# yzh119/custom_op_benchmark

Measured on AMD Instinct MI355X. Metric: edges/sec fwd+bwd (SDDMM+softmax+SpMM) on Reddit d=64; HBM GB/s vs roofline, higher is better.
Workload: dtype f32; 1 GPU; reddit-shape Chung-Lu(alpha=0.50) graph, N=232965 E=114615892 per GPU, h=1 d=64, U[0,1) values, chunk_size=32, int64 CSR both orientations; graph=reddit, nodes=232965, edges=114615892, heads=1, d=64, chunk_size=32, row_chunks=3694777, col_chunks=3694424, parallelism=single GPU

## Files before the change

### custom_op_benchmark_amd/_lib.py

```python
import atexit
import collections
import ctypes
import os
import weakref

import torch

_HERE = os.path.dirname(os.path.abspath(__file__))
LIB_PATH = os.environ.get("GRAPHOP_LIB") or os.path.join(_HERE, "libgraphop_hip.so")
ABI_VERSION = 8

F32, F64 = 0, 1
_c64 = ctypes.c_int64
_vp = ctypes.c_void_p
_lib = None


class PlanInfo(ctypes.Structure):
    _fields_ = [("n_chunks", _c64), ("n_edges", _c64), ("n_segments", _c64), ("max_row", _c64),
                ("max_index", _c64), ("max_segment_len", _c64), ("rows_sorted", ctypes.c_int32),
                ("indptr_monotone", ctypes.c_int32), ("eid_identity", ctypes.c_int32),
                ("full_coverage", ctypes.c_int32), ("row_owned", ctypes.c_int32),
                ("has_idx32", ctypes.c_int32), ("dense_fill_pct", ctypes.c_int32),
                ("sorted_in_rows", ctypes.c_int32), ("n_dense_blocks", _c64), ("max_row_gap", _c64),
                ("n_geometry_fallbacks", _c64),
                ("sddmm_tile_rows", ctypes.c_int32), ("sddmm_tile_repeat_permille", ctypes.c_int32),
                ("sddmm_tile_max_parts", ctypes.c_int32)]


class SweepInfo(ctypes.Structure):
    _fields_ = [("win_cols", _c64), ("W", ctypes.c_int32), ("T", ctypes.c_int32), ("V", ctypes.c_int32),
                ("n_dealt", ctypes.c_int32)]


ALLOC_FN = ctypes.CFUNCTYPE(ctypes.c_void_p, ctypes.c_size_t, ctypes.c_int, ctypes.c_void_p)
FREE_FN = ctypes.CFUNCTYPE(None, ctypes.c_void_p)


class ProfileRec(ctypes.Structure):
    _fields_ = [("name", ctypes.c_char * 48), ("kernel", ctypes.c_char * 48), ("calls", _c64), ("total_ms", ctypes.c_double),
                ("min_ms", ctypes.c_double), ("max_ms", ctypes.c_double)]


_P = _vp
_SIGNATURES = {
    "graphop_tune": [ctypes.c_char_p, ctypes.c_int],
    "graphop_tune_reset": [],
    "graphop_check_device_errors": [],
    "graphop_tune_get": [ctypes.c_char_p, ctypes.POINTER(ctypes.c_int)],
    "graphop_profile_enable": [ctypes.c_int],
    "graphop_profile_read": [ctypes.POINTER(ProfileRec), ctypes.c_int],
    "graphop_partition_csr_count": [_P, _c64, _c64, _P, _P],
    "graphop_partition_csr_fill": [_P, _P, _c64, _c64, _c64, _P, _P, _P],
    "graphop_plan_create": [_P, _P, _P, _P, _c64, _c64, _c64, _P, ctypes.POINTER(_vp)],
    "graphop_plan_info": [_P, ctypes.POINTER(PlanInfo)],
    "graphop_set_allocator": [ALLOC_FN, FREE_FN],
    "graphop_plan_prepare": [_P, ctypes.c_int, _c64, _c64, _c64, ctypes.c_int, _P],
    "graphop_plan_n_sweeps": [_P],
    "graphop_plan_sweep_info": [_P, ctypes.c_int, ctypes.POINTER(SweepInfo)],
    "graphop_plan_array": [_P, ctypes.c_char_p, ctypes.c_int, ctypes.POINTER(_vp), ctypes.POINTER(_c64)],
    "graphop_plan_import": [_P] * 4 + [ctypes.POINTER(PlanInfo)] + [_P] * 4 + [_c64] + [_P] * 4 + [ctypes.POINTER(_vp)],
    "graphop_plan_import_sweep": [_P, ctypes.POINTER(SweepInfo), _P, _P, _P, _P],
    "graphop_plan_sweep_dealt": [_P, ctypes.c_int, ctypes.c_int, ctypes.POINTER(ctypes.c_int32), ctypes.POINTER(ctypes.c_int32)],
    "graphop_plan_sweep_build_dealt": [_P, ctypes.POINTER(SweepInfo), ctypes.c_int32, ctypes.c_int32, _P],
    "graphop_maskedmm_csr_forward": [ctypes.c_int] + [_P] * 7 + [_c64] * 6 + [_P, _P],
    "graphop_maskedmm_csr_forward_partial": [ctypes.c_int] + [_P] * 7 + [_c64] * 7 + [_P],
    "graphop_maskedmm_csr_backward": [ctypes.c_int] + [_P] * 13 + [_c64] * 7 + [_P, _P, _P],
    "graphop_sparse_softmax_forward": [ctypes.c_int] + [_P] * 5 + [_c64] * 3 + [_P, _c64, _P, _P],
    "graphop_sparse_softmax_backward": [ctypes.c_int] + [_P] * 6 + [_c64] * 3 + [_P, _c64, _P, _P],
    "graphop_vector_spmm_forward": [ctypes.c_int] + [_P] * 7 + [_c64] * 6 + [_P, _P],
    "graphop_vector_spmm_backward": [ctypes.c_int] + [_P] * 13 + [_c64] * 7 + [_P, _P, _P],
    "graphop_spmm_pair_supported": [ctypes.c_int] + [_c64] * 5 + [_P],
    "graphop_spmm_pair": [ctypes.c_int] + [_P] * 9 + [_c64] * 6 + [_P, _P],
    "graphop_interleave_pairs": [ctypes.c_int, _P, _P, _P, _c64, _P],
    "graphop_node_mul_edge_forward": [ctypes.c_int] + [_P] * 6 + [_c64] * 5 + [_P, _P],
    "graphop_node_mul_edge_backward": [ctypes.c_int] + [_P] * 8 + [_c64] * 5 + [_P, _P],
    "graphop_gat_scores_forward": [ctypes.c_int] + [_P] * 7 + [_c64] * 5 + [ctypes.c_double, _P, _P],
    "graphop_gat_scores_backward": [ctypes.c_int] + [_P] * 13 + [_c64] * 6 + [ctypes.c_double, _P, _P, _P],
    "graphop_gatv2_scores_forward": [ctypes.c_int] + [_P] * 8 + [_c64] * 6 + [ctypes.c_double, _P, _P],
    "graphop_gatv2_scores_backward": [ctypes.c_int] + [_P] * 16 + [_c64] * 8 + [ctypes.c_double, _P, _P, _P],
    "graphop_gatv2_attention_forward": [ctypes.c_int] + [_P] * 9 + [_c64] * 6 + [ctypes.c_double, _P, _P],
    "graphop_gatv2_attention_backward": [ctypes.c_int] + [_P] * 18 + [_c64] * 8 + [ctypes.c_double, _P, _P, _P],
    "graphop_gatv2_attention_dropout_forward": [ctypes.c_int] + [_P] * 9 + [_c64] * 6
    + [ctypes.c_double, ctypes.c_double, ctypes.c_uint64, ctypes.c_uint32, _P, _P],
    "graphop_gatv2_attention_dropout_backward": [ctypes.c_int] + [_P] * 18 + [_c64] * 8
    + [ctypes.c_double, ctypes.c_double, ctypes.c_uint64, ctypes.c_uint32, _P, _P, _P],
    "graphop_gat_attention_forward": [ctypes.c_int] + [_P] * 9 + [_c64] * 6 + [ctypes.c_double, _P, _P],
    "graphop_gat_attention_backward": [ctypes.c_int] + [_P] * 18 + [_c64] * 8 + [ctypes.c_double, _P, _P, _P],
    "graphop_gat_attention_dropout_forward": [ctypes.c_int] + [_P] * 9 + [_c64] * 6
    + [ctypes.c_double, ctypes.c_double, ctypes.c_uint64, ctypes.c_uint32, _P, _P],
    "graphop_gat_attention_dropout_backward": [ctypes.c_int] + [_P] * 18 + [_c64] * 8
    + [ctypes.c_double, ctypes.c_double, ctypes.c_uint64, ctypes.c_uint32, _P, _P, _P],
    "graphop_edge_dropout_mask": [ctypes.c_int] + [_P] * 5 + [_c64] * 5
    + [ctypes.c_double, ctypes.c_uint64, ctypes.c_uint32, _P, _P],
    "graphop_gat_edge_attention_forward": [ctypes.c_int] + [_P] * 10 + [_c64] * 6
    + [ctypes.c_double, ctypes.c_double, ctypes.c_uint64, ctypes.c_uint32, _P, _P],
    "graphop_gat_edge_attention_backward": [ctypes.c_int] + [_P] * 20 + [_c64] * 8
    + [ctypes.c_double, ctypes.c_double, ctypes.c_uint64, ctypes.c_uint32, _P, _P, _P],
    "graphop_gatv2_edge_attention_forward": [ctypes.c_int] + [_P] * 10 + [_c64] * 6
    + [ctypes.c_double, ctypes.c_double, ctypes.c_uint64, ctypes.c_uint32, _P, _P],
    "graphop_gatv2_edge_attention_backward": [ctypes.c_int] + [_P] * 20 + [_c64] * 8
    + [ctypes.c_double, ctypes.c_double, ctypes.c_uint64, ctypes.c_uint32, _P, _P, _P],
    "graphop_gather_rows": [ctypes.c_int, _P, _P, _P, _c64, _c64, _c64, _P],
    "graphop_scatter_add_rows": [ctypes.c_int, _P, _P, _P, _c64, _c64, _c64, _P],
    "graphop_add_rows_unique": [ctypes.c_int, _P, _P, _P, _c64, _c64, _c64, _P],
    "graphop_add_rows_grouped": [ctypes.c_int, _P, _P, _P, _P, _P, _c64, _c64, _c64, _P],
    "graphop_attention_workspace_bytes": [ctypes.c_int, ctypes.c_int] + [_c64] * 5 + [_P, _P, _P,
                                                                                       ctypes.POINTER(_c64)],
    "graphop_attention_backward_is_fused": [ctypes.c_int] + [_c64] * 5 + [_P, _P, _P, ctypes.POINTER(ctypes.c_int)],
    "graphop_attention_forward": [ctypes.c_int] + [_P] * 9 + [_c64] * 6 + [_P, _c64, _P, _P],
    "graphop_attention_backward": [ctypes.c_int] + [_P] * 17 + [_c64] * 7 + [_P, _c64, _P, _P, _P],
    "graphop_attention_dropout_workspace_bytes": [ctypes.c_int, ctypes.c_int] + [_c64] * 5 + [_P, _P, _P,
                                                                                               ctypes.POINTER(_c64)],
    "graphop_attention_dropout_forward": [ctypes.c_int] + [_P] * 9 + [_c64] * 6 + [_P, _c64, _P, _P]
    + [ctypes.c_double, ctypes.c_uint64, ctypes.c_uint32, _c64],
    "graphop_attention_dropout_backward": [ctypes.c_int] + [_P] * 17 + [_c64] * 7 + [_P, _c64, _P, _P, _P]
    + [ctypes.c_double, ctypes.c_uint64, ctypes.c_uint32, _c64],
    "graphop_attention_bias_workspace_bytes": [ctypes.c_int, ctypes.c_int] + [_c64] * 5 + [_P, _P, _P, ctypes.c_int,
                                                                                            ctypes.POINTER(_c64)],
    "graphop_attention_bias_forward": [ctypes.c_int] + [_P] * 10 + [_c64] * 6 + [_P, _c64, _P, _P]
    + [ctypes.c_double, ctypes.c_uint64, ctypes.c_uint32, _c64],
    "graphop_attention_bias_backward": [ctypes.c_int] + [_P] * 19 + [_c64] * 7 + [_P, _c64, _P, _P, _P]
    + [ctypes.c_double, ctypes.c_uint64, ctypes.c_uint32, _c64],
    "graphop_attention_edge_workspace_bytes": [ctypes.c_int, ctypes.c_int] + [_c64] * 5 + [_P, _P, _P,
                                                                                            ctypes.POINTER(_c64)],
    "graphop_attention_edge_forward": [ctypes.c_int] + [_P] * 10 + [_c64] * 6 + [_P, _c64, _P, _P]
    + [ctypes.c_double, ctypes.c_uint64, ctypes.c_uint32, _c64],
    "graphop_attention_edge_backward": [ctypes.c_int] + [_P] * 19 + [_c64] * 7 + [_P, _c64, _P, _P, _P]
    + [ctypes.c_double, ctypes.c_uint64, ctypes.c_uint32, _c64],
    "graphop_attention_etype_workspace_bytes": [ctypes.c_int, ctypes.c_int] + [_c64] * 6 + [_P, _P, _P,
                                                                                             ctypes.POINTER(_c64)],
    "graphop_attention_etype_forward": [ctypes.c_int] + [_P] * 11 + [_c64] * 7 + [_P, _c64, _P, _P]
    + [ctypes.c_double, ctypes.c_uint64, ctypes.c_uint32, _c64],
    "graphop_attention_etype_backward": [ctypes.c_int] + [_P] * 20 + [_c64] * 8 + [_P, _c64, _P, _P, _P]
    + [ctypes.c_double, ctypes.c_uint64, ctypes.c_uint32, _c64],
    "graphop_attention_tbias_workspace_bytes": [ctypes.c_int, ctypes.c_int] + [_c64] * 6 + [_P, _P, _P,
                                                                                             ctypes.POINTER(_c64)],
    "graphop_attention_tbias_forward": [ctypes.c_int] + [_P] * 11 + [_c64] * 7 + [_P, _c64, _P, _P]
    + [ctypes.c_double, ctypes.c_uint64, ctypes.c_uint32, _c64],
    "graphop_attention_tbias_backward": [ctypes.c_int] + [_P] * 20 + [_c64] * 8 + [_P, _c64, _P, _P, _P]
    + [ctypes.c_double, ctypes.c_uint64, ctypes.c_uint32, _c64],
# ... 418 lines not shown
```

### custom_op_benchmark_amd/csrc/graphop_hip.hip

```cpp
#include <stdarg.h>

#include <map>
#include <mutex>
#include <set>
#include <string>
#include <vector>

#include "common.h"
#include "host.h"
#include "host_attn_rows.h"
#include "kernels_fast.h"
#include "kernels_walk.h"
#include "kernels_tile.h"
#include "tile_layout.h"
#include "kernels_attn_walk.h"
#include "kernels_attn_bias_fwd.h"
#include "kernels_block.h"
#include "kernels_attn.h"
#include "kernels_generic.h"

namespace graphop {

namespace {

// ... 361 lines not shown
    } else {
      allow_full_lds((const void*)k_attn_fwd_walk_f32<L, false>);
      hipLaunchKernelGGL((k_attn_fwd_walk_f32<L, false>), dim3(wl.blocks), dim3(kWalkThreads), lds_bytes, st, wl.view, a, NoDrop{});
    }
  }
  attn_pieces_merge(
      "attn_fwd_merge", "k_attn_piece_add", w, L, st,
      [&](dim3 grid, dim3 block) { hipLaunchKernelGGL(k_attn_piece_max, grid, block, 0, st, w.p_row, w.p_ml, w.Mtmp, w.np); },
      [&](dim3 grid, dim3 block) {
        hipLaunchKernelGGL((k_attn_piece_add<L>), grid, block, 0, st, w.p_row, w.p_ml, w.p_o, w.Mtmp, w.Ltmp, a.o, w.np);
      },
      [&](dim3 grid, dim3 block) {
        hipLaunchKernelGGL((k_attn_piece_fin<L>), grid, block, 0, st, w.p_row, w.Mtmp, w.Ltmp, a.o, a.stats, w.np);
      });
  if (hipGetLastError() != hipSuccess) return -GRAPHOP_ERR_HIP;
  return 1;
}

int attn_bias_fwd_rows(const Csr& g, i64 n_q, i64 n_k, i64 h, i64 d, int dtype, const void* Q, const void* K,
                       const void* V, const void* b, void* o, void* stats, void* ws, i64 ws_bytes, hipStream_t st,
                       bool dry_run, size_t* ws_needed, const AttnDrop* drop) {
  const Tuning& t = tuning();
  const graphop_plan* plan = g.plan;
  const i64 n_chunks = g.n_chunks, n_edges = g.n_edges;
  if (ws_needed) *ws_needed = 0;
  if (!t.attn_fused || !t.attn_rows || t.force_generic || dtype != GRAPHOP_F32 || h != 1 || !plan) return 0;
  if (d % 4 != 0 || !pow2(d) || d < 16 || d > 1024 || n_edges == 0 || n_chunks == 0) return 0;
  if (!g.owned() || !plan->indices) return 0;
  if (plan->info.max_row >= n_q || plan->info.max_index >= n_k || n_q >= kWalkRowMask) return 0;
  const i64 F = d;
  const ChunkGeometry geo = attn_one_head_geometry(n_chunks, F);
  if (2 * geo.groups >= 0x7fffffffLL) return 0;
  const AttnRowsFwdWs w(ws, 2 * geo.groups, n_q, 1, F);
  if (ws_needed) *ws_needed = w.total;
  if (dry_run) return 1;
  if (!ws || (size_t)ws_bytes < w.total) return 0;
  AttnBiasFwdArgs a;
  a.Q = (const float*)Q; a.K = (const float*)K; a.V = (const float*)V; a.b = (const float*)b;
  a.o = (float*)o; a.stats = (float*)stats;
  a.p_row = w.p_row; a.p_ml = w.p_ml; a.p_o = w.p_o;
  if (zero_async(o, sizeof(float) * (size_t)(n_q * F), st) != hipSuccess) return -GRAPHOP_ERR_HIP;
  attn_pieces_fill("attn_bias_fwd_setup", w, kAttnNegBig, st);
  const i64* eids = g.eid_or_null();
  {
    ProfScope prof("attn_bias_fwd_rows", st, drop ? "k_attn_bias_fwd_rows_f32<DROP>" : "k_attn_bias_fwd_rows_f32");
    GO_DISPATCH_LNV((int)F, {
      if (drop)
        hipLaunchKernelGGL((k_attn_bias_fwd_rows_f32<L, NV, true>), dim3(geo.blocks), dim3(kFastBlock), 0, st,
                           g.row, g.indptr, eids, g.indices, a, n_chunks,
                           (int)geo.cpg, *drop);
      else
        hipLaunchKernelGGL((k_attn_bias_fwd_rows_f32<L, NV, false>), dim3(geo.blocks), dim3(kFastBlock), 0, st,
                           g.row, g.indptr, eids, g.indices, a, n_chunks,
                           (int)geo.cpg, NoDrop{});
    });
  }
  attn_pieces_merge(
      "attn_bias_fwd_merge", "k_attn_bias_piece_add", w, geo.lanes, st,
      [&](dim3 grid, dim3 block) { hipLaunchKernelGGL(k_attn_piece_max, grid, block, 0, st, w.p_row, w.p_ml, w.Mtmp, w.np); },
      [&](dim3 grid, dim3 block) {
        GO_DISPATCH_LNV((int)F, {
          hipLaunchKernelGGL((k_attn_bias_piece_add<L, NV>), grid, block, 0, st, w.p_row, w.p_ml, w.p_o, w.Mtmp, w.Ltmp,
                             a.o, w.np);
        });
      },
      [&](dim3 grid, dim3 block) {
        GO_DISPATCH_LNV((int)F, {
          hipLaunchKernelGGL((k_attn_bias_piece_fin<L, NV>), grid, block, 0, st, w.p_row, w.Mtmp, w.Ltmp, a.o, a.stats,
                             w.np);
        });
      });
  if (hipGetLastError() != hipSuccess) return -GRAPHOP_ERR_HIP;
  return 1;
}

namespace {

struct TileLaunch {
  TileView view;
  unsigned blocks;
  size_t lds_bytes;
  int nt;
};
template <int L, int NV>
int choose_tile(const graphop_plan* plan, i64 n_table_rows, i64 h, int dtype, hipStream_t st, TileLaunch* out, bool dry_run) {
  if constexpr (L != 16 || NV != 1) {
    return 0;
  } else {
    const Tuning& t = tuning();
    if (!t.sddmm_tile || !plan || dtype != GRAPHOP_F32 || h != 1) return 0;
    if (!plan->info.eid_identity || !table_off32(n_table_rows, L, NV)) return 0;
    const int R = t.sddmm_tile_rows;
    if (R != 128 && R != 192 && R != 256 && R != 384) return 0;
    SweepLaunch sl;
    SweepOpts so;
    so.dry_run = 1;
    so.tile = 1;
    so.bpc = sweep_bpc(NV, true);
    const int use = choose_sweep(plan, n_table_rows, L, NV, st, &sl, false, &so);
    if (use != 1) return use;
    const int per_cu = R <= 192 ? 2 : 1;
    if (t.sddmm_tile != 2 && (i64)sl.sweep->W * ceil_div((i64)sl.sweep->V, R) < 32LL * t.n_cu * per_cu) return 0;
    const int lds_wg = (kTileLdsBytes / per_cu) & ~255;
    int cap = (lds_wg - R * 16 * L * NV) / 4;
    if (cap > kTileMaxCap) cap = kTileMaxCap;
    const Sweep::Tile* tl = nullptr;
    const int rc = plan_get_tile(const_cast<graphop_plan*>(plan), sl.sweep, R, cap, t.sddmm_tile == 2, t.sddmm_tile_min_repeat, st, &tl);
    if (rc != GRAPHOP_OK) return -rc;
    if (!tl) return 0;
    plan_trim(const_cast<graphop_plan*>(plan));
    TileView& v = out->view;
    v = TileView{};
    v.part_ptr = tl->part_ptr; v.parts = (const int4*)tl->parts; v.rec = tl->rec; v.bstart = tl->bstart; v.slotw = tl->slotw;
    v.rowtab = (const int2*)tl->rowtab; v.tdesc = (const int4*)tl->tdesc; v.vr_row = sl.sweep->vr_row;
    v.V = sl.sweep->V; v.W = sl.sweep->W; v.R = R; v.tiles = tl->tiles; v.win_cols = (int)sl.sweep->win_cols;
    v.touch = t.sddmm_tile_touch ? 1 : 0;
    v.sync = nullptr;
    if (!dry_run) {
      v.sync = plan_take_queue(const_cast<graphop_plan*>(plan), sl.sweep);
      if (zero_async(v.sync, sizeof(int) * kQueueInts, st) != hipSuccess) return -GRAPHOP_ERR_HIP;
    }
    const i64 tasks = (i64)tl->tiles * v.W;
    i64 nb = (i64)t.n_cu * per_cu;
    if (nb > tasks) nb = tasks;
    out->blocks = (unsigned)(nb < 1 ? 1 : nb);
    out->lds_bytes = (size_t)R * 16 * L * NV + (size_t)cap * 4;
    out->nt = per_cu == 2 ? 512 : 1024;
    return 1;
  }
}
template <int L, int NV>
void launch_tile(const TileLaunch& tl, const float* a, const float* b, float* y, hipStream_t st) {
  if constexpr (L == 16 && NV == 1) {
    if (tl.nt == 512) {
      allow_full_lds((const void*)k_sddmm_tile_f32<L, NV, 512>);
      hipLaunchKernelGGL((k_sddmm_tile_f32<L, NV, 512>), dim3(tl.blocks), dim3(512), tl.lds_bytes, st, tl.view, a, b, y);
    } else {
      allow_full_lds((const void*)k_sddmm_tile_f32<L, NV, 1024>);
      hipLaunchKernelGGL((k_sddmm_tile_f32<L, NV, 1024>), dim3(tl.blocks), dim3(1024), tl.lds_bytes, st, tl.view, a, b, y);
    }
  }
}

template <int L, int NV>
int try_sddmm_sweep(const char* tag, int dtype, const graphop_plan* plan, i64 n_table_rows, const void* A,
                    const void* B, void* y, i64 h, int d4, hipStream_t st) {
  if (!plan) return 0;
  {
    TileLaunch tl;
    const int ut = choose_tile<L, NV>(plan, n_table_rows, h, dtype, st, &tl, false);
    if (ut < 0) return ut;
    if (ut == 1) {
      ProfScope prof(tag, st, "k_sddmm_tile_f32");
      launch_tile<L, NV>(tl, (const float*)A, (const float*)B, (float*)y, st);
      return 1;
    }
  }
  SweepLaunch sl;
  SweepOpts so;
  const bool f64 = dtype == GRAPHOP_F64;
  if (f64 && (h != 1 || NV != 1 || L < 16 || !sddmm_staged(plan, L, NV, h, n_table_rows))) return 0;
  const bool off32 = table_off32(n_table_rows, L, NV);
  so.bpc = (f64 || !off32) ? 3 : sweep_bpc(NV, h == 1);
  so.touch = tuning().touch_sddmm;
  const bool id = plan->info.eid_identity != 0;
  so.staged = sddmm_staged(plan, L, NV, h, n_table_rows);
  so.stage_lds_per_group = StageCfg<L, 1>::kLdsIntsPerGroup * (int)sizeof(int) + (h > 1 ? 64 * (int)h : 0);
  if (h > 1 && !aligned16(y)) so.staged = false;
  const int use = choose_sweep(plan, n_table_rows, L, NV, st, &sl, false, &so);
  if (use != 1) return use;
  const bool staged = sl.view.rec != nullptr;
  if (f64 && !staged) return 0;
  ProfScope prof(tag, st, f64 ? "k_sddmm_wown_staged_f64" : staged ? "k_sddmm_wown_staged_f32" : "k_sddmm_wown_f32");
  const dim3 grid(sl.blocks), block(kFastBlock);
  if (f64) {
    if constexpr (NV == 1 && L >= 16) {
      if (off32) hipLaunchKernelGGL((k_sddmm_wown_staged_f64<L, NV, true>), grid, block, sl.lds_bytes, st, sl.view,
                                    (const double*)A, (const double*)B, (double*)y);
      else hipLaunchKernelGGL((k_sddmm_wown_staged_f64<L, NV, false>), grid, block, sl.lds_bytes, st, sl.view,
                              (const double*)A, (const double*)B, (double*)y);
    }
    return 1;
  }
  const float* a = (const float*)A;
  const float* b = (const float*)B;
  float* yy = (float*)y;
  if (staged) {
    if (h == 1) {
      if (off32) hipLaunchKernelGGL((k_sddmm_wown_staged_f32<L, NV, 0, true>), grid, block, sl.lds_bytes, st, sl.view, a, b, yy);
      else hipLaunchKernelGGL((k_sddmm_wown_staged_f32<L, NV, 0, false>), grid, block, sl.lds_bytes, st, sl.view, a, b, yy);
    } else if constexpr (NV == 1 && L >= 16) {
      auto go = [&](auto dc) {
        constexpr int D4 = decltype(dc)::value;
        if constexpr (D4 < L)
          hipLaunchKernelGGL((k_sddmm_wown_staged_f32<L, NV, D4>), grid, block, sl.lds_bytes, st, sl.view, a, b, yy);
      };
      switch (d4) {
        case 4: go(std::integral_constant<int, 4>{}); break;
        case 8: go(std::integral_constant<int, 8>{}); break;
        case 16: go(std::integral_constant<int, 16>{}); break;
        default: go(std::integral_constant<int, 32>{}); break;
      }
    }
    return 1;
  }
#define GO_K(H1, ID, O32)                                                                      \
  hipLaunchKernelGGL((k_sddmm_wown_f32<L, NV, H1, ID, O32>), grid, block, sl.lds_bytes, st,    \
                     sl.view, a, b, yy, (int)h, d4)
  if (h == 1) {
    if (id) { if (off32) GO_K(true, true, true); else GO_K(true, true, false); }
    else { if (off32) GO_K(true, false, true); else GO_K(true, false, false); }
  } else {
    if (id) GO_K(false, true, false); else GO_K(false, false, false);
  }
#undef GO_K
  return 1;
}

template <int L, int NV>
int try_spmm_sweep(const char* tag, const graphop_plan* plan, i64 n_table_rows, const void* w,
                   const void* X, void* out, i64 h, int d4, hipStream_t st) {
  SweepLaunch sl;
// ... 382 lines not shown
  GO_LAUNCH_CHECK();
  return GRAPHOP_OK;
}

template <typename T>
int softmax_forward_t(const Csr& g, const T* x, T* y, i64 h, T* ws, i64 ws_rows, hipStream_t st, T* stats = nullptr) {
  const i64 *row = g.row, *indptr = g.indptr, *eid = g.eid;
  const i64 C = g.n_chunks, E = g.n_edges;
  const graphop_plan* plan = g.plan_slots;
  const bool owned = plan && plan->info.row_owned;
  const bool covered = owned && plan->info.full_coverage && plan->info.eid_identity;
  if (!covered && E * h > 0) GO_HIP(zero_async(y, sizeof(T) * (size_t)(E * h), st));
  if (C == 0) return GRAPHOP_OK;
  if (owned) return launch_softmax_seg<T, false>(g, x, (const T*)nullptr, y, h, st, stats);
  GO_CHECK_ARG(ws != nullptr && ws_rows > 0,
               "sparse_softmax_forward: the general (plan-less) path needs a workspace of "
               "2*workspace_rows*h values with workspace_rows > max(row)");
  T* max_val = ws;
  T* sum = ws + ws_rows * h;
  const unsigned fb = (unsigned)ceil_div(ws_rows * h, 256) > 4096u ? 4096u
                                                                   : (unsigned)ceil_div(ws_rows * h, 256);
  hipLaunchKernelGGL((k_fill<T>), dim3(fb), dim3(256), 0, st, max_val, ws_rows * h, (T)-1e9);
  GO_HIP(zero_async(sum, sizeof(T) * (size_t)(ws_rows * h), st));
  const unsigned nb = blocks_for(C, kGenericWavesPerBlock);
  hipLaunchKernelGGL((k_softmax_max<T>), dim3(nb), dim3(kGenericBlock), 0, st, row, indptr, eid, x,
                     max_val, C, h);
  hipLaunchKernelGGL((k_softmax_exp_sum<T>), dim3(nb), dim3(kGenericBlock), 0, st, row, indptr,
                     eid, x, (const T*)max_val, sum, y, C, h);
  hipLaunchKernelGGL((k_softmax_norm<T>), dim3(nb), dim3(kGenericBlock), 0, st, row, indptr, eid,
                     (const T*)sum, y, C, h);
  if (stats)
    hipLaunchKernelGGL((k_attn_stats_from_ws<T>), dim3(fb), dim3(256), 0, st, (const T*)max_val,
                       (const T*)sum, stats, ws_rows * h);
  GO_LAUNCH_CHECK();
  return GRAPHOP_OK;
}

template <typename T>
int softmax_backward_t(const Csr& g, const T* y, const T* dy, T* dx, i64 h, T* ws, i64 ws_rows, hipStream_t st) {
  const i64 *row = g.row, *indptr = g.indptr, *eid = g.eid;
  const i64 C = g.n_chunks, E = g.n_edges;
  const graphop_plan* plan = g.plan_slots;
  const bool owned = plan && plan->info.row_owned;
  const bool covered = owned && plan->info.full_coverage && plan->info.eid_identity;
  if (!covered && E * h > 0) GO_HIP(zero_async(dx, sizeof(T) * (size_t)(E * h), st));
  if (C == 0) return GRAPHOP_OK;
  if (owned) return launch_softmax_seg<T, true>(g, y, dy, dx, h, st);
  GO_CHECK_ARG(ws != nullptr && ws_rows > 0,
               "sparse_softmax_backward: the general (plan-less) path needs a workspace of "
               "workspace_rows*h values with workspace_rows > max(row)");
  GO_HIP(zero_async(ws, sizeof(T) * (size_t)(ws_rows * h), st));
  const unsigned nb = blocks_for(C, kGenericWavesPerBlock);
  hipLaunchKernelGGL((k_softmax_bwd_aggre<T>), dim3(nb), dim3(kGenericBlock), 0, st, row, indptr,
                     eid, dy, y, ws, C, h);
  hipLaunchKernelGGL((k_softmax_bwd_dx<T>), dim3(nb), dim3(kGenericBlock), 0, st, row, indptr, eid,
                     dy, y, (const T*)ws, dx, C, h);
  GO_LAUNCH_CHECK();
  return GRAPHOP_OK;
}

inline int check_common(const char* fn, int dtype, i64 C, i64 E, i64 h, i64 d) {
  GO_TRY(check_async_error(false));
  GO_CHECK_ARG(dtype == GRAPHOP_F32 || dtype == GRAPHOP_F64, "%s: dtype must be GRAPHOP_F32 or "
               "GRAPHOP_F64", fn);
  GO_CHECK_ARG(C >= 0 && E >= 0 && h >= 1 && d >= 0, "%s: negative size (n_chunks=%lld n_edges=%lld "
               "h=%lld d=%lld)", fn, (long long)C, (long long)E, (long long)h, (long long)d);
  return GRAPHOP_OK;
}

}

int softmax_forward_stats(int dtype, const Csr& g, const void* x, void* y, i64 h, void* ws, i64 ws_rows, hipStream_t st,
                          void* stats) {
  if (dtype == GRAPHOP_F32)
    return softmax_forward_t<float>(g, (const float*)x, (float*)y, h, (float*)ws, ws_rows, st, (float*)stats);
  return softmax_forward_t<double>(g, (const double*)x, (double*)y, h, (double*)ws, ws_rows, st, (double*)stats);
}
}

using namespace graphop;

extern "C" {

int graphop_plan_prepare(graphop_plan_t* plan, int dtype, int64_t n_table_rows, int64_t h, int64_t d,
                         int fused, void* stream) {
  GO_CHECK_ARG(plan != nullptr && n_table_rows >= 0 && h >= 1 && d >= 0, "plan_prepare: bad arguments");
  hipStream_t st = (hipStream_t)stream;
  const bool f64 = fast64_ok(dtype, h, d, plan->info.n_edges, n_table_rows);
  if (!f64 && !fast_ok(dtype, h, d, plan->info.n_edges, n_table_rows)) return GRAPHOP_OK;
  int rc = 0;
  GO_DISPATCH_LNV((int)(f64 ? 2 * d : h * d), {
    SweepLaunch sl;
    SweepOpts o;
    o.dry_run = 1;
    o.bpc = f64 ? 3 : sweep_bpc(NV, h == 1);
    o.staged = sddmm_staged(plan, L, NV, h, n_table_rows);
    o.stage_lds_per_group = StageCfg<L, 1>::kLdsIntsPerGroup * (int)sizeof(int) + (h > 1 ? 64 * (int)h : 0);
    int tiled = 0;
    if (!f64) {
      TileLaunch tl;
      tiled = choose_tile<L, NV>(plan, n_table_rows, h, dtype, st, &tl, true);
      if (tiled < 0) rc = tiled;
    }
    if (tiled == 0 && (!f64 || (o.staged && NV == 1 && L >= 16)))
      rc = choose_sweep(plan, n_table_rows, L, NV, st, &sl, false, &o);
    o.staged = spmm_staged(L, NV, h, n_table_rows);
    if (rc >= 0 && !f64) rc = choose_sweep(plan, n_table_rows, L, NV, st, &sl, true, &o);
    if constexpr (NV == 1 && L >= 16) {
      WalkLaunch wl;
      const int bit = plan->info.eid_identity ? 2 : 4;
      const int K = spmm_walk_k<L, NV>(h, dtype);
      if (rc >= 0 && K > 0 && (tuning().walk & bit) && (h == 1 || table_off32(n_table_rows, L, NV))) {
        const int r2 = choose_walk<L, NV>(plan, n_table_rows, K, st, &wl, true);
        if (r2 < 0) rc = r2;
      }
    }
  });
  if (rc < 0) return -rc;
  if (fused && h == 1) {
    rc = 0;
    if (fused != 3) {
      const int fw = attn_fwd_walk(plan, plan->info.max_row + 1, n_table_rows, h, d, dtype, nullptr, nullptr, nullptr, nullptr,
                                   nullptr, nullptr, 0, st, true, nullptr);
      if (fw < 0) return -fw;
    }
    if (fused != 3) rc = attn_prepare_plan(plan, n_table_rows, d, false, st);
    if (rc >= 0 && fused != 2) rc = attn_prepare_plan(plan, n_table_rows, d, true, st);
    if (rc < 0) return -rc;
  }
  return GRAPHOP_OK;
}

int graphop_maskedmm_csr_forward(int dtype, const int64_t* row, const int64_t* indptr,
                                 const int64_t* eid, const int64_t* indices, const void* A,
                                 const void* B, void* y, int64_t n_chunks, int64_t n_edges,
                                 int64_t n_a, int64_t n_b, int64_t h, int64_t d,
                                 const graphop_plan_t* plan, void* stream) {
  const char* fn = "maskedmm_csr_forward";
  GO_TRY(check_common(fn, dtype, n_chunks, n_edges, h, d));
  hipStream_t st = (hipStream_t)stream;
  if (n_edges * h == 0) return GRAPHOP_OK;
  GO_PTR(fn, y);
  const Csr g(row, indptr, eid, indices, n_chunks, n_edges, plan);
  if (!g.covered(true)) GO_HIP(zero_async(y, esize(dtype) * (size_t)(n_edges * h), st));
  if (n_chunks == 0) return GRAPHOP_OK;
  GO_TRY(g.require(fn)); GO_PTR(fn, A); GO_PTR(fn, B);
  GO_TRY(Csr::check_bounds(fn, g.plan_slots, "A", n_a, nullptr, 0));
  GO_TRY(Csr::check_bounds(fn, g.plan, "A", n_a, "B", n_b));
  return launch_sddmm<false>("sddmm_fwd", dtype, g, A, B, y, n_b, h, d, st);
}

int graphop_maskedmm_csr_forward_partial(int dtype, const int64_t* row, const int64_t* indptr,
                                         const int64_t* eid, const int64_t* indices, const void* A,
                                         const void* B, void* y, int64_t n_chunks, int64_t n_slots,
                                         int64_t n_y, int64_t n_a, int64_t n_b, int64_t h, int64_t d,
                                         void* stream) {
  const char* fn = "maskedmm_csr_forward_partial";
  GO_TRY(check_common(fn, dtype, n_chunks, n_slots, h, d));
  GO_CHECK_ARG(n_y >= n_slots && n_a >= 0 && n_b >= 0, "%s: n_y (%lld) must be at least n_slots (%lld): eid[] names distinct "
               "entries of y", fn, (long long)n_y, (long long)n_slots);
  hipStream_t st = (hipStream_t)stream;
  if (n_slots * h == 0 || n_chunks == 0) return GRAPHOP_OK;
  const Csr g(row, indptr, eid, indices, n_chunks, n_y, nullptr);
  GO_PTR(fn, y); GO_TRY(g.require(fn)); GO_PTR(fn, A); GO_PTR(fn, B);
  return launch_sddmm<false>("sddmm_fwd_part", dtype, g, A, B, y, n_b, h, d, st);
}
// ... 277 lines not shown
```

### custom_op_benchmark_amd/csrc/kernels_tile.h

```cpp
#pragma once
#include "kernels_wown.h"

namespace graphop {

struct TileView {
  const int* part_ptr;
  const int4* parts;
  const unsigned short* rec;
  const int* bstart;
  const int* slotw;
  const int2* rowtab;
  const int4* tdesc;
  const int* vr_row;
  int* sync;
  int V, W, R, tiles;
  int win_cols;
  int touch;
};

constexpr int kTileLdsBytes = 158 * 1024;

__device__ __forceinline__ int row16_incl_scan(int v) {
  v += __builtin_amdgcn_update_dpp(0, v, 0x111, 0xF, 0xF, true);
  v += __builtin_amdgcn_update_dpp(0, v, 0x112, 0xF, 0xF, true);
  v += __builtin_amdgcn_update_dpp(0, v, 0x114, 0xF, 0xF, true);
  v += __builtin_amdgcn_update_dpp(0, v, 0x118, 0xF, 0xF, true);
  return v;
}
__device__ __forceinline__ int row16_max(int v) {
  v = max(v, __builtin_amdgcn_update_dpp(0, v, 0xB1, 0xF, 0xF, true));
  v = max(v, __builtin_amdgcn_update_dpp(0, v, 0x4E, 0xF, 0xF, true));
  v = max(v, __builtin_amdgcn_update_dpp(0, v, 0x141, 0xF, 0xF, true));
  v = max(v, __builtin_amdgcn_update_dpp(0, v, 0x140, 0xF, 0xF, true));
  return v;
}

constexpr int kTileDescParts = 4;

template <int L = 16, int NV = 1, int NT = 1024>
__global__ __launch_bounds__(NT, 4) void k_sddmm_tile_f32(TileView tv, const float* __restrict__ A,
                                                          const float* __restrict__ B, float* __restrict__ y) {
  static_assert(L == 16 && NV == 1, "256-B rows: one float4 per lane of a 16-lane group");
  extern __shared__ float4 lds[];
  __shared__ int task_sh[2][2];
  __shared__ int desc_sh[2][2 + 4 * kTileDescParts];
  __shared__ int ctr_sh;
  constexpr int G = NT / L;
  const int l = threadIdx.x % L, g = threadIdx.x / L;
  float* res = reinterpret_cast<float*>(lds + (i64)tv.R * L);
  const char* lds_l = reinterpret_cast<const char*>(lds) + l * 16;
  SweepView qv{};
  qv.sync = tv.sync;
  qv.W = tv.W;
  WownQueue queue(qv, tv.tiles);
  auto fetch_desc = [&](int slot, int w, int t) {
    const int lane = threadIdx.x & (kWave - 1);
    const i64 task = (i64)w * tv.tiles + t;
    const int p0 = tv.part_ptr[task], p1 = tv.part_ptr[task + 1];
    if (lane < 4 * kTileDescParts && p0 * 4 + lane < p1 * 4)
      desc_sh[slot][2 + lane] = reinterpret_cast<const int*>(tv.parts)[(i64)p0 * 4 + lane];
    if (lane == 0) { desc_sh[slot][0] = p0; desc_sh[slot][1] = p1; }
  };
  int raw = -1;
  if (threadIdx.x < kWave) {
    int w = -1, t = 0;
    const bool more = queue.pull(w, t);
    raw = more ? queue.issue() : -1;
    if (threadIdx.x == 0) { task_sh[0][0] = more ? w : -1; task_sh[0][1] = t; }
    if (more) fetch_desc(0, w, t);
  }
  auto next_batch = [&]() {
    int v = 0;
    if (l == 0) v = atomicAdd(&ctr_sh, 1);
    return group_bcast<L, 0>(v);
  };
  int par = 0;
  for (;;) {
    __syncthreads();
    const int w = task_sh[par][0], t = task_sh[par][1];
    if (w < 0) break;
    if (threadIdx.x < kWave) {
      int wn = -1, tn = 0;
      const bool more = queue.resolve(raw, wn, tn);
      raw = more ? queue.issue() : -1;
      if (threadIdx.x == 0) { task_sh[par ^ 1][0] = more ? wn : -1; task_sh[par ^ 1][1] = tn; }
    }
    if (threadIdx.x == kWave) ctr_sh = 0;
    const int v0 = t * tv.R;
    const int nr = (tv.V - v0) < tv.R ? (tv.V - v0) : tv.R;
    const int2* rows = tv.rowtab + ((i64)w * tv.V + v0);
    for (int i = g; i < nr; i += G) {
      const int2 r = rows[i];
      const i64 arow = tv.vr_row[v0 + i];
      if (((unsigned)r.y >> 16) != 0) lds[i * L + l] = ld4(A, arow * L + l);
    }
    __syncthreads();
    if (threadIdx.x >= NT - kWave) {
      const int wn = task_sh[par ^ 1][0], tn = task_sh[par ^ 1][1];
      if (wn >= 0) {
        fetch_desc(par ^ 1, wn, tn);
        if (tv.touch) {
          const int4 nd = tv.tdesc[(i64)wn * tv.tiles + tn];
          const int lane = threadIdx.x & (kWave - 1);
          int tch[11];
#pragma unroll
          for (int q = 0; q < 11; ++q) tch[q] = 0;
          const int nrec = nd.y * 16;
#pragma unroll
          for (int q = 0; q < 3; ++q) {
            const int at = (q * kWave + lane) * 64;
            if (at < nrec) tch[q] = tv.rec[(i64)nd.x * 16 + at];
          }
#pragma unroll
          for (int q = 0; q < 5; ++q) {
            const int at = (q * kWave + lane) * 32;
            if (at < nd.w) tch[3 + q] = tv.slotw[(i64)nd.z + at];
          }
          if (lane * 32 < nd.y) tch[8] = tv.bstart[nd.x + lane * 32];
          const int vn = tn * tv.R;
          const int nrn = (tv.V - vn) < tv.R ? (tv.V - vn) : tv.R;
          if (lane * 16 < nrn) tch[9] = tv.rowtab[(i64)wn * tv.V + vn + lane * 16].x;
          if (lane * 32 < nrn) tch[10] = tv.vr_row[vn + lane * 32];
          asm volatile("; touched %0 %1 %2 %3 %4 %5 %6 %7 %8 %9 %10" ::"v"(tch[0]), "v"(tch[1]), "v"(tch[2]), "v"(tch[3]),
                       "v"(tch[4]), "v"(tch[5]), "v"(tch[6]), "v"(tch[7]), "v"(tch[8]), "v"(tch[9]), "v"(tch[10]));
        }
      }
    }
    const unsigned win_id0 = (unsigned)w * (unsigned)tv.win_cols;
    const int p0 = desc_sh[par][0], p1 = desc_sh[par][1];
    for (int p = p0; p < p1; ++p) {
      int4 pt;
      if (p - p0 < kTileDescParts) {
        const int* d = &desc_sh[par][2 + 4 * (p - p0)];
        pt = make_int4(d[0], d[1], d[2], d[3]);
      } else {
        pt = tv.parts[p];
      }
      const int nb = (pt.y + 15) >> 4;
      int b = next_batch();
      int rw = 0, bs = 0;
      if (b < nb) { rw = tv.rec[((i64)pt.x + b) * 16 + l]; bs = tv.bstart[(i64)pt.x + b]; }
      while (b < nb) {
        const bool valid = b * 16 + l < pt.y;
        const int cnt = valid ? (rw & 3) + 1 : 0;
        const unsigned my_off = valid ? (win_id0 + (unsigned)(rw >> 2)) * 256u : 0u;
        const int first = bs + row16_incl_scan(cnt) - cnt;
        const int gmax = row16_max(cnt);
        int sw[4];
#pragma unroll
        for (int k = 0; k < 4; ++k) {
          sw[k] = 0;
          if (__builtin_amdgcn_ballot_w64(k < cnt) != 0 && k < cnt) sw[k] = tv.slotw[first + k];
        }
        float4 bb[16];
        static_for<16>([&](auto uc) {
          constexpr int u = decltype(uc)::value;
          const unsigned o = group_bcast<L, u>(my_off);
          bb[u] = ld16_off<float>(B, o + (unsigned)(l * 16));
        });
        const int bn = next_batch();
        if (bn < nb) { rw = tv.rec[((i64)pt.x + bn) * 16 + l]; bs = tv.bstart[(i64)pt.x + bn]; }
#pragma unroll
        for (int k = 0; k < 4; ++k) {
          if (k < gmax) {
            const unsigned my_koff = ((unsigned)sw[k] >> 16) * 256u;
            float part[16];
            static_for<16>([&](auto uc) {
              constexpr int u = decltype(uc)::value;
              const unsigned ko = group_bcast<L, u>(my_koff);
              const float4 av = *reinterpret_cast<const float4*>(lds_l + ko);
              part[u] = dot4(av, bb[u]);
            });
            const float r = group_dots_to_owner<L, 16>(part, l);
            if (k < cnt) res[sw[k] & 0xffff] = r;
          }
        }
        b = bn;
      }
      __syncthreads();
      if (threadIdx.x == kWave) ctr_sh = 0;
      for (int i = pt.z + g; i < pt.z + pt.w; i += G) {
        const int2 r = rows[i];
        const int len = (int)((unsigned)r.y >> 16), off = r.y & 0xffff;
        for (int x = l; x < len; x += L) __builtin_nontemporal_store(res[off + x], y + ((i64)r.x + x));
      }
      if (p + 1 < p1) __syncthreads();
    }
    par ^= 1;
  }
}

}
```

### include/graphop_hip.h

```cpp
#ifndef GRAPHOP_HIP_H_
#define GRAPHOP_HIP_H_

#include <stddef.h>
#include <stdint.h>

#ifdef __cplusplus
extern "C" {
#endif

#if defined(__GNUC__)
#define GRAPHOP_API __attribute__((visibility("default")))
#else
#define GRAPHOP_API
#endif

#define GRAPHOP_ABI_VERSION 8

#define GRAPHOP_F32 0
#define GRAPHOP_F64 1

#define GRAPHOP_OK 0
#define GRAPHOP_ERR_INVALID_ARGUMENT 1
#define GRAPHOP_ERR_HIP 2
#define GRAPHOP_ERR_BAD_GRAPH 3

typedef struct graphop_plan graphop_plan_t;

typedef struct graphop_plan_info {
  int64_t n_chunks;
  int64_t n_edges;
  int64_t n_segments;
  int64_t max_row;
  int64_t max_index;
  int64_t max_segment_len;
  int32_t rows_sorted;
  int32_t indptr_monotone;
  int32_t eid_identity;
  int32_t full_coverage;
  int32_t row_owned;
  int32_t has_idx32;
  int32_t dense_fill_pct;
  int32_t sorted_in_rows;
  int64_t n_dense_blocks;
  int64_t max_row_gap;
  int64_t n_geometry_fallbacks;
  int32_t sddmm_tile_rows;
  int32_t sddmm_tile_repeat_permille;
  int32_t sddmm_tile_max_parts;
} graphop_plan_info_t;

GRAPHOP_API int graphop_abi_version(void);
GRAPHOP_API const char* graphop_last_error(void);
GRAPHOP_API int graphop_check_device_errors(void);

GRAPHOP_API int graphop_tune(const char* key, int value);
GRAPHOP_API int graphop_tune_reset(void);
GRAPHOP_API int graphop_tune_get(const char* key, int* value);
GRAPHOP_API const char* graphop_tune_key(int i);
GRAPHOP_API int64_t graphop_memory_bytes(void);

typedef void* (*graphop_alloc_fn)(size_t bytes, int device, void* stream);
typedef void (*graphop_free_fn)(void* ptr);
GRAPHOP_API int graphop_set_allocator(graphop_alloc_fn alloc_fn, graphop_free_fn free_fn);

typedef struct graphop_profile_rec {
  char name[48];
  char kernel[48];
  int64_t calls;
  double total_ms;
  double min_ms;
  double max_ms;
} graphop_profile_rec_t;
GRAPHOP_API int graphop_profile_enable(int on);
GRAPHOP_API int graphop_profile_read(graphop_profile_rec_t* out, int cap);

GRAPHOP_API int graphop_partition_csr_count(const int64_t* indptr, int64_t n_rows, int64_t chunk_size,
                                int64_t* first_chunk, void* stream);
GRAPHOP_API int graphop_partition_csr_fill(const int64_t* indptr, const int64_t* first_chunk, int64_t n_rows,
                               int64_t chunk_size, int64_t n_chunks, int64_t* row,
                               int64_t* indptr_out, void* stream);

GRAPHOP_API int graphop_plan_create(const int64_t* row, const int64_t* indptr, const int64_t* eid,
                        const int64_t* indices, int64_t n_chunks, int64_t n_edges,
                        int64_t n_index_bound, void* stream, graphop_plan_t** plan_out);
GRAPHOP_API int graphop_plan_info(const graphop_plan_t* plan, graphop_plan_info_t* info_out);
GRAPHOP_API void graphop_plan_destroy(graphop_plan_t* plan);

GRAPHOP_API int graphop_plan_prepare(graphop_plan_t* plan, int dtype, int64_t n_table_rows, int64_t h,
                         int64_t d, int fused, void* stream);

typedef struct graphop_sweep_info {
  int64_t win_cols;
  int32_t W;
  int32_t T;
  int32_t V;
  int32_t n_dealt;
} graphop_sweep_info_t;
GRAPHOP_API int graphop_plan_n_sweeps(const graphop_plan_t* plan);
GRAPHOP_API int graphop_plan_sweep_info(const graphop_plan_t* plan, int sweep, graphop_sweep_info_t* out);
GRAPHOP_API int graphop_plan_array(const graphop_plan_t* plan, const char* name, int sweep, const void** ptr,
                       int64_t* bytes);
GRAPHOP_API int graphop_plan_import(const int64_t* row, const int64_t* indptr, const int64_t* eid,
                        const int64_t* indices, const graphop_plan_info_t* info,
                        const int64_t* seg_chunk, const int32_t* idx32, const int32_t* eid32,
                        const int32_t* long_segs, int64_t n_long, const int32_t* blk_seg,
                        const int32_t* seg_e0, const int32_t* seg_row, void* stream,
                        graphop_plan_t** plan_out);
GRAPHOP_API int graphop_plan_import_sweep(graphop_plan_t* plan, const graphop_sweep_info_t* info,
                              const int32_t* vr_row, const int32_t* wp_lo, const int32_t* wp_hi,
                              void* stream);
GRAPHOP_API int graphop_plan_sweep_dealt(const graphop_plan_t* plan, int sweep, int i, int32_t* L, int32_t* K);
GRAPHOP_API int graphop_plan_sweep_build_dealt(graphop_plan_t* plan, const graphop_sweep_info_t* info, int32_t L,
                                   int32_t K, void* stream);

GRAPHOP_API int graphop_maskedmm_csr_forward(int dtype, const int64_t* row, const int64_t* indptr,
                                 const int64_t* eid, const int64_t* indices, const void* A,
                                 const void* B, void* y, int64_t n_chunks, int64_t n_edges,
                                 int64_t n_a, int64_t n_b, int64_t h, int64_t d,
                                 const graphop_plan_t* plan, void* stream);

GRAPHOP_API int graphop_maskedmm_csr_forward_partial(int dtype, const int64_t* row, const int64_t* indptr,
                                         const int64_t* eid, const int64_t* indices, const void* A,
                                         const void* B, void* y, int64_t n_chunks, int64_t n_slots,
                                         int64_t n_y, int64_t n_a, int64_t n_b, int64_t h, int64_t d,
                                         void* stream);

GRAPHOP_API int graphop_maskedmm_csr_backward(int dtype, const int64_t* row, const int64_t* indptr_r,
                                  const int64_t* eid_r, const int64_t* indices_r,
                                  const int64_t* col, const int64_t* indptr_c,
                                  const int64_t* eid_c, const int64_t* indices_c, const void* A,
                                  const void* B, const void* dy, void* dA, void* dB,
                                  int64_t n_row_chunks, int64_t n_col_chunks, int64_t n_edges,
                                  int64_t n_a, int64_t n_b, int64_t h, int64_t d,
                                  const graphop_plan_t* plan_r, const graphop_plan_t* plan_c,
                                  void* stream);

GRAPHOP_API int graphop_sparse_softmax_forward(int dtype, const int64_t* row, const int64_t* indptr,
                                   const int64_t* eid, const void* x, void* y, int64_t n_chunks,
                                   int64_t n_edges, int64_t h, void* workspace,
                                   int64_t workspace_rows, const graphop_plan_t* plan,
                                   void* stream);

// ... 295 lines not shown
```

Baseline: 10.27 billion edges/s.

## Load SDDMM tile rows straight into LDS and batch row-table reads per group

The tile SDDMM kernel now stages A rows into LDS with global_load_lds direct-to-LDS loads instead of going through registers. Each group lane fetches the row-table entry and source row index up front, and group broadcasts then drive the loads and the final scatter stores. R becomes a compile-time template parameter (rows per group times groups), the part descriptor is made wave-uniform with readfirstlane, and a C entry point exposes the computed LDS capacity. The intent is to cut VGPR traffic and serialized per-row index loads in the staging and writeback phases. The cost is more template instantiations and a dependence on the LDS layout matching the direct-load addressing.

```diff
diff --git a/custom_op_benchmark_amd/_lib.py b/custom_op_benchmark_amd/_lib.py
--- a/custom_op_benchmark_amd/_lib.py
+++ b/custom_op_benchmark_amd/_lib.py
@@ -57,6 +57,7 @@
     "graphop_set_allocator": [ALLOC_FN, FREE_FN],
     "graphop_plan_prepare": [_P, ctypes.c_int, _c64, _c64, _c64, ctypes.c_int, _P],
     "graphop_plan_n_sweeps": [_P],
+    "graphop_sddmm_tile_cap": [ctypes.c_int],
     "graphop_plan_sweep_info": [_P, ctypes.c_int, ctypes.POINTER(SweepInfo)],
     "graphop_plan_array": [_P, ctypes.c_char_p, ctypes.c_int, ctypes.POINTER(_vp), ctypes.POINTER(_c64)],
     "graphop_plan_import": [_P] * 4 + [ctypes.POINTER(PlanInfo)] + [_P] * 4 + [_c64] + [_P] * 4 + [ctypes.POINTER(_vp)],
diff --git a/custom_op_benchmark_amd/csrc/graphop_hip.hip b/custom_op_benchmark_amd/csrc/graphop_hip.hip
--- a/custom_op_benchmark_amd/csrc/graphop_hip.hip
+++ b/custom_op_benchmark_amd/csrc/graphop_hip.hip
@@ -467,6 +467,13 @@
   size_t lds_bytes;
   int nt;
 };
+int tile_per_cu(int R) { return (R == 128 || R == 192) ? 2 : (R == 256 || R == 384) ? 1 : 0; }
+int tile_cap(int R) {
+  const int per_cu = tile_per_cu(R);
+  if (!per_cu) return 0;
+  const int cap = (((kTileLdsBytes / per_cu) & ~255) - R * 256) / 4;
+  return cap > kTileMaxCap ? kTileMaxCap : cap;
+}
 template <int L, int NV>
 int choose_tile(const graphop_plan* plan, i64 n_table_rows, i64 h, int dtype, hipStream_t st, TileLaunch* out, bool dry_run) {
   if constexpr (L != 16 || NV != 1) {
@@ -476,7 +483,8 @@
     if (!t.sddmm_tile || !plan || dtype != GRAPHOP_F32 || h != 1) return 0;
     if (!plan->info.eid_identity || !table_off32(n_table_rows, L, NV)) return 0;
     const int R = t.sddmm_tile_rows;
-    if (R != 128 && R != 192 && R != 256 && R != 384) return 0;
+    const int per_cu = tile_per_cu(R);
+    if (!per_cu) return 0;
     SweepLaunch sl;
     SweepOpts so;
     so.dry_run = 1;
@@ -484,11 +492,8 @@
     so.bpc = sweep_bpc(NV, true);
     const int use = choose_sweep(plan, n_table_rows, L, NV, st, &sl, false, &so);
     if (use != 1) return use;
-    const int per_cu = R <= 192 ? 2 : 1;
     if (t.sddmm_tile != 2 && (i64)sl.sweep->W * ceil_div((i64)sl.sweep->V, R) < 32LL * t.n_cu * per_cu) return 0;
-    const int lds_wg = (kTileLdsBytes / per_cu) & ~255;
-    int cap = (lds_wg - R * 16 * L * NV) / 4;
-    if (cap > kTileMaxCap) cap = kTileMaxCap;
+    const int cap = tile_cap(R);
     const Sweep::Tile* tl = nullptr;
     const int rc = plan_get_tile(const_cast<graphop_plan*>(plan), sl.sweep, R, cap, t.sddmm_tile == 2, t.sddmm_tile_min_repeat, st, &tl);
     if (rc != GRAPHOP_OK) return -rc;
@@ -517,12 +522,18 @@
 template <int L, int NV>
 void launch_tile(const TileLaunch& tl, const float* a, const float* b, float* y, hipStream_t st) {
   if constexpr (L == 16 && NV == 1) {
-    if (tl.nt == 512) {
-      allow_full_lds((const void*)k_sddmm_tile_f32<L, NV, 512>);
-      hipLaunchKernelGGL((k_sddmm_tile_f32<L, NV, 512>), dim3(tl.blocks), dim3(512), tl.lds_bytes, st, tl.view, a, b, y);
-    } else {
-      allow_full_lds((const void*)k_sddmm_tile_f32<L, NV, 1024>);
-      hipLaunchKernelGGL((k_sddmm_tile_f32<L, NV, 1024>), dim3(tl.blocks), dim3(1024), tl.lds_bytes, st, tl.view, a, b, y);
+    auto go = [&](auto ntc, auto rpgc) {
+      constexpr int NT = decltype(ntc)::value, RPG = decltype(rpgc)::value;
+      allow_full_lds((const void*)k_sddmm_tile_f32<L, NV, NT, RPG>);
+      hipLaunchKernelGGL((k_sddmm_tile_f32<L, NV, NT, RPG>), dim3(tl.blocks), dim3(NT), tl.lds_bytes, st, tl.view, a, b, y);
+    };
+    using std::integral_constant;
+    switch (tl.view.R) {
+      case 128: go(integral_constant<int, 512>{}, integral_constant<int, 4>{}); break;
+      case 192: go(integral_constant<int, 512>{}, integral_constant<int, 6>{}); break;
+      case 256: go(integral_constant<int, 1024>{}, integral_constant<int, 4>{}); break;
+      case 384: go(integral_constant<int, 1024>{}, integral_constant<int, 6>{}); break;
+      default: break;
     }
   }
 }
@@ -1071,6 +1082,8 @@
 
 extern "C" {
 
+int graphop_sddmm_tile_cap(int rows) { return tile_cap(rows); }
+
 int graphop_plan_prepare(graphop_plan_t* plan, int dtype, int64_t n_table_rows, int64_t h, int64_t d,
                          int fused, void* stream) {
   GO_CHECK_ARG(plan != nullptr && n_table_rows >= 0 && h >= 1 && d >= 0, "plan_prepare: bad arguments");
diff --git a/custom_op_benchmark_amd/csrc/kernels_tile.h b/custom_op_benchmark_amd/csrc/kernels_tile.h
--- a/custom_op_benchmark_amd/csrc/kernels_tile.h
+++ b/custom_op_benchmark_amd/csrc/kernels_tile.h
@@ -35,19 +35,27 @@
   return v;
 }
 
+__device__ __forceinline__ void ld16_to_lds(const float* src, float4* wave_base) {
+  __builtin_amdgcn_global_load_lds((const __attribute__((address_space(1))) void*)src,
+                                   (__attribute__((address_space(3))) void*)wave_base, 16, 0, 0);
+}
+__device__ __forceinline__ void wait_vmem() { __builtin_amdgcn_s_waitcnt(0x0F70); }
+
 constexpr int kTileDescParts = 4;
 
-template <int L = 16, int NV = 1, int NT = 1024>
+template <int L = 16, int NV = 1, int NT = 1024, int RPG = 4>
 __global__ __launch_bounds__(NT, 4) void k_sddmm_tile_f32(TileView tv, const float* __restrict__ A,
                                                           const float* __restrict__ B, float* __restrict__ y) {
   static_assert(L == 16 && NV == 1, "256-B rows: one float4 per lane of a 16-lane group");
+  static_assert(RPG >= 1 && RPG <= L, "one lane of a group per vrow entry");
   extern __shared__ float4 lds[];
   __shared__ int task_sh[2][2];
   __shared__ int desc_sh[2][2 + 4 * kTileDescParts];
   __shared__ int ctr_sh;
   constexpr int G = NT / L;
+  constexpr int R = RPG * G;
   const int l = threadIdx.x % L, g = threadIdx.x / L;
-  float* res = reinterpret_cast<float*>(lds + (i64)tv.R * L);
+  float* res = reinterpret_cast<float*>(lds + R * L);
   const char* lds_l = reinterpret_cast<const char*>(lds) + l * 16;
   SweepView qv{};
   qv.sync = tv.sync;
@@ -86,14 +94,24 @@
       if (threadIdx.x == 0) { task_sh[par ^ 1][0] = more ? wn : -1; task_sh[par ^ 1][1] = tn; }
     }
     if (threadIdx.x == kWave) ctr_sh = 0;
-    const int v0 = t * tv.R;
-    const int nr = (tv.V - v0) < tv.R ? (tv.V - v0) : tv.R;
+    const int v0 = t * R;
+    const int nr = (tv.V - v0) < R ? (tv.V - v0) : R;
     const int2* rows = tv.rowtab + ((i64)w * tv.V + v0);
-    for (int i = g; i < nr; i += G) {
-      const int2 r = rows[i];
-      const i64 arow = tv.vr_row[v0 + i];
-      if (((unsigned)r.y >> 16) != 0) lds[i * L + l] = ld4(A, arow * L + l);
-    }
+    {
+      const int mine = g + l * G;
+      int ey = 0, ar = 0;
+      if (l < RPG && mine < nr) {
+        ey = rows[mine].y;
+        ar = tv.vr_row[v0 + mine];
+      }
+      float4* const wave_rows = lds + (threadIdx.x / kWave) * (kWave / L) * L;
+      static_for<RPG>([&](auto jc) {
+        constexpr int j = decltype(jc)::value;
+        const i64 arow = group_bcast<L, j>(ar);
+        if (((unsigned)group_bcast<L, j>(ey) >> 16) != 0) ld16_to_lds(A + (arow * L + l) * 4, wave_rows + j * G * L);
+      });
+    }
+    wait_vmem();
     __syncthreads();
     if (threadIdx.x >= NT - kWave) {
       const int wn = task_sh[par ^ 1][0], tn = task_sh[par ^ 1][1];
@@ -117,8 +135,8 @@
             if (at < nd.w) tch[3 + q] = tv.slotw[(i64)nd.z + at];
           }
           if (lane * 32 < nd.y) tch[8] = tv.bstart[nd.x + lane * 32];
-          const int vn = tn * tv.R;
-          const int nrn = (tv.V - vn) < tv.R ? (tv.V - vn) : tv.R;
+          const int vn = tn * R;
+          const int nrn = (tv.V - vn) < R ? (tv.V - vn) : R;
           if (lane * 16 < nrn) tch[9] = tv.rowtab[(i64)wn * tv.V + vn + lane * 16].x;
           if (lane * 32 < nrn) tch[10] = tv.vr_row[vn + lane * 32];
           asm volatile("; touched %0 %1 %2 %3 %4 %5 %6 %7 %8 %9 %10" ::"v"(tch[0]), "v"(tch[1]), "v"(tch[2]), "v"(tch[3]),
@@ -136,6 +154,8 @@
       } else {
         pt = tv.parts[p];
       }
+      pt = make_int4(__builtin_amdgcn_readfirstlane(pt.x), __builtin_amdgcn_readfirstlane(pt.y),
+                     __builtin_amdgcn_readfirstlane(pt.z), __builtin_amdgcn_readfirstlane(pt.w));
       const int nb = (pt.y + 15) >> 4;
       int b = next_batch();
       int rw = 0, bs = 0;
@@ -177,13 +197,16 @@
         }
         b = bn;
       }
+      int2 ent = make_int2(0, 0);
+      if (l < RPG && g + l * G < pt.w) ent = rows[pt.z + g + l * G];
       __syncthreads();
       if (threadIdx.x == kWave) ctr_sh = 0;
-      for (int i = pt.z + g; i < pt.z + pt.w; i += G) {
-        const int2 r = rows[i];
-        const int len = (int)((unsigned)r.y >> 16), off = r.y & 0xffff;
-        for (int x = l; x < len; x += L) __builtin_nontemporal_store(res[off + x], y + ((i64)r.x + x));
-      }
+      static_for<RPG>([&](auto kc) {
+        constexpr int k = decltype(kc)::value;
+        const int first = group_bcast<L, k>(ent.x), ry = group_bcast<L, k>(ent.y);
+        const int len = (int)((unsigned)ry >> 16), off = ry & 0xffff;
+        for (int x = l; x < len; x += L) __builtin_nontemporal_store(res[off + x], y + ((i64)first + x));
+      });
       if (p + 1 < p1) __syncthreads();
     }
     par ^= 1;
diff --git a/include/graphop_hip.h b/include/graphop_hip.h
--- a/include/graphop_hip.h
+++ b/include/graphop_hip.h
@@ -58,6 +58,7 @@
 GRAPHOP_API int graphop_tune_get(const char* key, int* value);
 GRAPHOP_API const char* graphop_tune_key(int i);
 GRAPHOP_API int64_t graphop_memory_bytes(void);
+GRAPHOP_API int graphop_sddmm_tile_cap(int rows);
 
 typedef void* (*graphop_alloc_fn)(size_t bytes, int device, void* stream);
 typedef void (*graphop_free_fn)(void* ptr);
```

After: 10.55 billion edges/s, median of 6. 2.7% higher.
